# fdb/frequensea

Hardware: AMD Instinct MI355X
Metric: fft_frames_per_sec_n8192 (higher is better)
Workload: dtype f32

## Files before the change

### frequensea_amd/csrc/fsea_fft_core.h

```cpp
#pragma once

#include <hip/hip_runtime.h>
#include <stddef.h>
#include <stdint.h>

#include <fsea_pk_asm.h>
#include "fsea_opt.h"
#ifdef FSEA_TUNE
#include <fsea_pk_asm_tune.h>
#endif

namespace fsea {

constexpr int ilog2c(int n) {
    int l = 0;
    while ((1 << l) < n) ++l;
    return l;
}

constexpr int bitrev_c(int i, int bits) {
    int r = 0;
    for (int b = 0; b < bits; ++b) {
        if (i & (1 << b)) r |= 1 << (bits - 1 - b);
    }
// ... 187 lines not shown
#endif

template <int N_, int T_, int FPW_, int WPE_, int NP_, int R0_, int R1_, int R2_ = 1, int R3_ = 1,
          bool TWL_ = true, bool TWR_ = true, int ABL_ = 0, int OPT_ = FSEA_DEFAULT_OPT>
struct FftCfg {
    static constexpr int OPT = OPT_;
    static constexpr int ABL = ABL_;
    static constexpr int N = N_, T = T_, FPW = FPW_, NP = NP_;
    static constexpr int WPE = WPE_;
    static constexpr int P = N_ / T_;
    static constexpr int WG = T_ * FPW_;
    static constexpr bool TWL = TWL_, TWR = TWR_;
    static constexpr int R(int i) { return i == 0 ? R0_ : i == 1 ? R1_ : i == 2 ? R2_ : R3_; }
    static constexpr int C(int i) { return P / R(i); }
    static constexpr int Ns(int i) { return i == 0 ? 1 : Ns(i - 1) * R(i - 1); }
    static constexpr int tw_len(int i) { return i == 0 ? 0 : (R(i) - 1) * Ns(i); }
    static constexpr int pad(int idx) { return lds_pad<N_ / T_>(idx); }
    static constexpr int LDS_FRAME = N_ + 2 * T_;
    static constexpr int lds_tw_off(int i) {
        return i <= 1 ? FPW_ * LDS_FRAME : lds_tw_off(i - 1) + tw_len(i - 1);
    }
    static constexpr int TAB_MID = lds_tw_off(NP_ - 1) - FPW_ * LDS_FRAME;
    static constexpr int TAB_HI = N_ >= 64 ? N_ / 64 : 1, TAB_LO = 64;
    static constexpr int TAB_SMALL = TAB_MID + (TWR_ ? TAB_HI + TAB_LO : 0);
    static constexpr int LDS_HI = FPW_ * LDS_FRAME + TAB_MID;
    static constexpr int LDS_LO = LDS_HI + TAB_HI;
    static constexpr int LDS_TOTAL = FPW_ * LDS_FRAME + ((TWL_ || TWR_) ? TAB_SMALL : 0);
    static constexpr int LDS_ALLOC = LDS_TOTAL + 2;
    static_assert(R0_ * R1_ * R2_ * R3_ == N_, "radices must multiply to N");
    static_assert(N_ % T_ == 0, "T must divide N");
    static_assert(NP_ >= 2 && NP_ <= 4, "2..4 passes");
};

struct FftArgs {
    const void *in;
    void *out;
    size_t n_frames;
    size_t hop;
    uint32_t xormask;
    int mode;
    unsigned *ctr;
    unsigned long long *trace;
    const cf *tw[4];
    const cf *tw_small;
    const cf *tw_def;
    double rot_delta, rot_phase0;
    cf rot_row[32];
    uint32_t tile_rows = 0, pitch_row = 0, pitch_tile = 0;
    size_t out_span = 0;
    uint32_t dynamic_units = 1;
    uint32_t run_len = 0;
    const float *win = nullptr;
    const cf *win_dc = nullptr;
    uint32_t win_offset = 0;
};

template <int C>
__device__ __forceinline__ void ld_c(const cf *p, cf *dst) {
    if constexpr (C == 1) {
        dst[0] = *p;
    } else {
#pragma unroll
        for (int c = 0; c < C; c += 2) {
            const cf2 q = *reinterpret_cast<const cf2 *>(p + c);
            dst[c] = cf{q[0], q[1]};
            dst[c + 1] = cf{q[2], q[3]};
        }
    }
}

template <int C>
__device__ __forceinline__ void st_c(cf *p, const cf *src) {
    if constexpr (C == 1) {
        *p = src[0];
    } else {
#pragma unroll
        for (int c = 0; c < C; c += 2) {
            *reinterpret_cast<cf2 *>(p + c) = cf2{src[c][0], src[c][1], src[c + 1][0], src[c + 1][1]};
        }
    }
}

typedef __amdgpu_buffer_rsrc_t rsrc_t;

__device__ __forceinline__ rsrc_t buffer_window(const void *base, size_t off, size_t total) {
    const size_t rem = total > off ? total - off : 0;
    char *p = const_cast<char *>(static_cast<const char *>(base)) + (rem ? off : 0);
    return __builtin_amdgcn_make_buffer_rsrc(p, 0, rem > 0xffffffffull ? 0xffffffffu : (uint32_t)rem, 0x00020000);
// ... 517 lines not shown
            const auto q = __builtin_amdgcn_raw_buffer_load_b128(rs, voff, (uint32_t)(16 * T * i), 0);
            wv[2 * i] = cf{u2f(q[0]), u2f(q[1])};
            wv[2 * i + 1] = cf{u2f(q[2]), u2f(q[3])};
        }
    }
    static constexpr bool BALANCE = WIN == 0 && !LATE_LOAD && !ROT && IN == IN_U8 &&
                                    (((MODE_T == MODE_DB5_U8_DCFIX || MODE_T == MODE_DB10_U8) && (Cfg::OPT & opt::BALANCE_PX) != 0) ||
                                     (MODE_T == MODE_MAG && (Cfg::OPT & opt::BALANCE_MAG) != 0));
    static constexpr int BALANCE_STORES = 32;
    static __device__ __forceinline__ void balance_vmcnt() {
        if constexpr (BALANCE) {
            const rsrc_t nowhere = buffer_window(nullptr, 0, 0);
#pragma unroll
            for (int i = 0; i < BALANCE_STORES; ++i) {
                __builtin_amdgcn_raw_buffer_store_b32(0u, nowhere, (uint32_t)(64 * i), 0u, 0);
            }
        }
    }
    template <bool OFFSET>
    static __device__ __forceinline__ void convert_windowed(const Raw *raw, uint32_t xormask, int t, cf *v) {
#pragma unroll
        for (int r = 0; r < R0; ++r) convert_row<IN, C0, false, OFFSET>(raw[r], OFFSET ? xormask ^ 0x80808080u : xormask, C0 * t, v + r * C0);
    }
    template <int C = 0>
    static __device__ __forceinline__ void pass0_windowed(cf *v, const cf *wv) {
        if constexpr (C < C0) {
            dft_regs_win<R0, C0, C>(v + C, wv);
            pass0_windowed<C + 1>(v, wv);
        }
    }

#ifdef FSEA_TUNE
#include "fsea_fft_tune_members.h"
    static __device__ __forceinline__ void run(const FftArgs &a, cf *lds_all) {
        if constexpr (W64) run_w64(a, lds_all);
        else if constexpr (V2) run_v2(a, lds_all);
        else run_v1(a, lds_all);
    }
#else
    static __device__ __forceinline__ void run(const FftArgs &a, cf *lds_all) { run_v1(a, lds_all); }
#endif

    static __device__ __forceinline__ void run_v1(const FftArgs &a, cf *lds_all) {
        const int tid = threadIdx.x;
        const int slot = (FPW == 1) ? 0 : tid / T;
        const int t = (FPW == 1) ? tid : tid % T;
        cf *lds = lds_all + slot * Cfg::LDS_FRAME;
        unsigned *tk = reinterpret_cast<unsigned *>(lds_all + Cfg::LDS_TOTAL);

        const unsigned b = blockIdx.x;
        const bool issuer = (tid == 0);
        const size_t n_units = RUNS ? (a.n_frames + a.run_len - 1) / a.run_len : (a.n_frames + FPW - 1) / FPW;
        Pools pools;
        pools.n_units = (unsigned)n_units;
        pools.grid = gridDim.x;
        unsigned cur = b % POOLS;

        if ((FSEA_TRACE != 0) && a.trace != nullptr && tid == 0) {
            const unsigned hw_id = read_hw_id(), xcc_id = read_xcc_id();
            a.trace[32 * b + 0] = wall_clock64();
            a.trace[32 * b + 2] = __builtin_readcyclecounter();
            a.trace[32 * b + 4] = hw_id;
            a.trace[32 * b + 5] = xcc_id;
        }

        const int mode = (MODE_T >= 0) ? MODE_T : a.mode;
        const uint32_t xormask = (MODE_T >= 0) ? 0u : a.xormask;
        const uint32_t esz = elem_bytes(mode);
        const size_t total_in = (size_t)IN_BPS * ((a.n_frames - 1) * a.hop + (size_t)N);
        const bool tiled = a.tile_rows != 0;
        const size_t total_out = (size_t)esz * (tiled ? a.out_span : a.n_frames * (size_t)N);
        const uint32_t in_voff = (uint32_t)IN_BPS * ((uint32_t)slot * (uint32_t)a.hop + (uint32_t)(C0 * t));
        const int tl = pass_lane<LAST>(t);
        const uint32_t out_elem = (uint32_t)slot * (tiled ? a.pitch_row : (uint32_t)N) + (uint32_t)(CL * tl);
        auto row_elem = [&](size_t f) -> size_t {
            if (!tiled) return f * (size_t)N;
            const uint32_t k = (uint32_t)f / a.tile_rows, y = (uint32_t)f - k * a.tile_rows;
            return (size_t)y * a.pitch_row + (size_t)k * a.pitch_tile;
        };

        size_t u = b;
#if FSEA_STATIC_CONTIG
        [[maybe_unused]] const size_t contig_per = (n_units + gridDim.x - 1) / gridDim.x;
        [[maybe_unused]] size_t contig_end = n_units;
        if constexpr (!RUNS) {
            u = (size_t)b * contig_per;
            contig_end = u + contig_per < n_units ? u + contig_per : n_units;
            if (u >= n_units) u = n_units;
        }
#endif
        unsigned tick_next = 0;
        const bool dyn = !RUNS && DYNAMIC && a.dynamic_units != 0;
        [[maybe_unused]] size_t fcur = RUNS ? (size_t)b * a.run_len : 0;
        [[maybe_unused]] unsigned jpos = 0;
        if (dyn) {
            u = (size_t)pools.start(cur) + b / POOLS;
            if (u >= pools.start(cur + 1)) u = n_units;
        }
        constexpr int TAB_COPY = (Cfg::TWL || Cfg::TWR) ? Cfg::TAB_SMALL : 0;
        constexpr int TAB_REGS = (TAB_COPY + Cfg::WG - 1) / Cfg::WG;
        cf tabv[TAB_REGS > 0 ? TAB_REGS : 1];
#pragma unroll
        for (int i = 0; i < TAB_REGS; ++i) {
            const int e = tid + i * Cfg::WG;
            tabv[i] = a.tw_small[e < TAB_COPY ? e : TAB_COPY - 1];
        }
        constexpr int R1 = Cfg::R(1), C1 = Cfg::C(1), Ns1 = Cfg::Ns(1);
        cf tw1[DEFER ? C1 * (R1 / 2) : 1];
        if constexpr (DEFER) {
            const int t1 = pass_lane<1>(t);
#pragma unroll
            for (int c = 0; c < C1; ++c) ld_c<R1 / 2>(a.tw_def + ((C1 * t1 + c) % Ns1) * (R1 / 2), tw1 + c * (R1 / 2));
        }
        [[maybe_unused]] const rsrc_t win_rs = buffer_window(WIN ? a.win : nullptr, 0, WIN ? (size_t)N * 4u : 0);
        cf wv[WPAIRS];
        cf dcv[(WIN_DC && !DC_IN_REGS) ? DC_REGS : 1];
        cf dcr[DC_IN_REGS ? 2 * CL : 1];
        if constexpr (DC_IN_REGS) {
#pragma unroll
            for (int c = 0; c < CL; ++c) {
                dcr[c] = a.win_dc[CL * tl + c];
                dcr[CL + c] = a.win_dc[NsL + CL * tl + c];
            }
        }
        if constexpr (WIN != 0) load_window(win_rs, t, wv);
        if constexpr (WIN_DC && !DC_IN_REGS) {
#pragma unroll
            for (int i = 0; i < DC_REGS; ++i) {
                const int e = tid + i * Cfg::WG;
                dcv[i] = a.win_dc[e < 2 * NsL ? e : 2 * NsL - 1];
            }
        }
        if (dyn) {
            if (issuer) tick_next = atomicAdd(a.ctr + 32 * cur, 1u);
        }
        Raw raw[R0];
        load_raw(buffer_window(a.in, (size_t)IN_BPS * (RUNS ? fcur : u * FPW) * a.hop, u < n_units ? total_in : 0), in_voff, raw);
        balance_vmcnt();

        if constexpr (TAB_COPY > 0) {
#pragma unroll
            for (int i = 0; i < TAB_REGS; ++i) {
                const int e = tid + i * Cfg::WG;
                lds_all[FPW * Cfg::LDS_FRAME + (e < TAB_COPY ? e : TAB_COPY - 1)] = tabv[i];
            }
            if constexpr (WIN_DC && !DC_IN_REGS) {
#pragma unroll
                for (int i = 0; i < DC_REGS; ++i) {
                    const int e = tid + i * Cfg::WG;
                    lds_all[DC_OFF + (e < 2 * NsL ? e : 2 * NsL - 1)] = dcv[i];
                }
            }
            if ((FSEA_TRACE != 0) && a.trace != nullptr && tid == 0) a.trace[32 * b + 28] = wall_clock64();
            __syncthreads();
            if ((FSEA_TRACE != 0) && a.trace != nullptr && tid == 0) a.trace[32 * b + 29] = wall_clock64();
        }
        cf twl[Cfg::TWR ? (RL - 1) * CL : 1];
        if constexpr (Cfg::TWR) {
            const cf *hi = lds_all + Cfg::LDS_HI, *lo = lds_all + Cfg::LDS_LO;
            auto root = [&](unsigned m) -> cf { return pk_cmul(hi[m >> 6], lo[m & 63u]); };
            constexpr int RB = RL >= 16 ? 8 : (RL >= 4 ? 2 : RL);
            constexpr int RA = RL / RB;
#pragma unroll
            for (int c = 0; c < CL; ++c) {
                const unsigned k = (unsigned)(CL * tl + c);
                cf wb[RB], wa[RA];
#pragma unroll
                for (int bb = 1; bb < RB; ++bb) wb[bb] = root((unsigned)bb * k);
#pragma unroll
                for (int aa = 1; aa < RA; ++aa) wa[aa] = root((unsigned)(RB * aa) * k);
#pragma unroll
// ... 62 lines not shown
                    convert_row<IN, C0, false>(raw[r], a.xormask, C0 * t, v + r * C0);
                    const cf wr = a.rot_row[r];
#pragma unroll
                    for (int c = 0; c < C0; ++c) {
                        v[r * C0 + c] = pk_cmul(v[r * C0 + c] + cf{128.0f, 128.0f}, pk_cmul_uniform(fr[c], wr));
                        if constexpr (WIN != 0) {
                            if (a.win_offset != 0) v[r * C0 + c] += cf{128.0f, 128.0f};
                        }
                    }
                }
            } else if constexpr (WIN != 0 && IN == IN_F32) {
#pragma unroll
                for (int r = 0; r < R0; ++r) convert_row<IN, C0, false>(raw[r], 0u, C0 * t, v + r * C0);
            } else if constexpr (WIN != 0) {
                if (a.win_offset != 0) convert_windowed<true>(raw, xormask, t, v);
                else convert_windowed<false>(raw, xormask, t, v);
            } else {
#pragma unroll
                for (int r = 0; r < R0; ++r) convert_row<IN, C0>(raw[r], xormask, C0 * t, v + r * C0);
            }
            if ((FSEA_TRACE != 0) && a.trace != nullptr && tid == 0 && iter == 0) {
                asm volatile("" ::"v"(v[0]));
                a.trace[32 * b + 30] = wall_clock64();
            }
            if constexpr (WIN != 0) {
                pass0_windowed(v, wv);
            } else {
#pragma unroll
                for (int c = 0; c < C0; ++c) dft_regs<R0, C0, (Cfg::ABL & abl::NO_FLOPS) != 0>(v + c);
            }
            lds_write<0>(lds, v, t);
            frame_sync();
            if ((FSEA_TRACE != 0) && a.trace != nullptr && tid == 0 && iter == 0) a.trace[32 * b + 7] = wall_clock64();
            size_t un = u + gridDim.x;
#if FSEA_STATIC_CONTIG
            if constexpr (!RUNS) un = u + 1 < contig_end ? u + 1 : n_units;
#endif
            [[maybe_unused]] size_t fnext = 0;
            [[maybe_unused]] bool same_run = false;
            if constexpr (RUNS) {
                same_run = (jpos + 1 < a.run_len) && (fcur + 1 < a.n_frames);
                un = same_run ? u : u + gridDim.x;
                fnext = same_run ? fcur + 1 : un * (size_t)a.run_len;
            }
            if (dyn) {
                if constexpr (Cfg::ABL & abl::NO_LDS) __syncthreads();
                const unsigned nu = __builtin_amdgcn_readfirstlane(tk[par]);
                par ^= 1u;
                un = (nu == NO_UNIT) ? n_units : (size_t)nu;
            }
            if constexpr (RUNS) {
                const rsrc_t rs = buffer_window(a.in, (size_t)IN_BPS * fnext * a.hop, un < n_units ? total_in : 0);
                if (same_run) {
#pragma unroll
                    for (int r = 0; r < R0 / 2; ++r) raw[r] = raw[r + R0 / 2];
                    load_raw_rows<R0 / 2, R0>(rs, in_voff, raw);
                } else {
                    load_raw(rs, in_voff, raw);
                }
            } else if constexpr ((Cfg::ABL & abl::NO_LOADS) == 0 && !LATE_LOAD) {
                load_raw(buffer_window(a.in, (size_t)IN_BPS * (un * FPW) * a.hop, un < n_units ? total_in : 0), in_voff, raw);
            }
            middle_pass<1>(lds, lds_all, v, a, t, tw1);

            lds_read<LAST>(lds, v, tl);
            after_reads();
            frame_sync();
            if constexpr (Cfg::TWR && TW_FUSE) {
#pragma unroll
                for (int c = 0; c < CL; ++c) dft_regs_tw<RL, CL, CL>(v + c, twl + c, PRESCALED ? SC : 1.0f);
            } else if constexpr (Cfg::TWR) {
                if constexpr (PRESCALED) {
#pragma unroll
                    for (int c = 0; c < CL; ++c) v[c] = v[c] * cf{SC, SC};
                }
// ... 25 lines not shown
                for (int c = 0; c < CL; c += CB) {
                    cf dc_lo[CB], dc_hi[CB];
                    ld_c<CB>(lds_all + DC_OFF + CL * tl + c, dc_lo);
                    ld_c<CB>(lds_all + DC_OFF + NsL + CL * tl + c, dc_hi);
#pragma unroll
                    for (int j = 0; j < CB; ++j) {
                        v[(RL / 2 - 1) * CL + c + j] += dc_lo[j];
                        v[(RL / 2) * CL + c + j] += dc_hi[j];
                    }
                }
            }
            if constexpr (WIN != 0) {
                if constexpr (WIN == 1) {
                    load_window(win_rs, t, wv);
                    __builtin_amdgcn_sched_barrier(0);
                }
            }
            epilogue(mode, buffer_window(a.out, (size_t)esz * row_elem(RUNS ? fcur : u * FPW), total_out), out_elem, v, tl);
            if constexpr (LATE_LOAD) {
                load_raw(buffer_window(a.in, (size_t)IN_BPS * (un * FPW) * a.hop, un < n_units ? total_in : 0), in_voff, raw);
            }
            u = un;
            if constexpr (RUNS) {
                fcur = fnext;
                jpos = same_run ? jpos + 1 : 0;
            }
            if ((FSEA_TRACE != 0) && a.trace != nullptr && tid == 0 && iter < 24) a.trace[32 * b + 8 + iter] = wall_clock64();
            ++iter;
        }

        if (dyn && issuer) {
            __builtin_amdgcn_s_waitcnt(0);
            const unsigned finished = atomicAdd(a.ctr + 32 * POOLS, 1u);
            if (finished == gridDim.x - 1) {
#pragma unroll
                for (unsigned q = 0; q <= POOLS; ++q) a.ctr[32 * q] = 0;
            }
        }
        if ((FSEA_TRACE != 0) && a.trace != nullptr && tid == 0) {
            a.trace[32 * b + 1] = wall_clock64();
            a.trace[32 * b + 3] = __builtin_readcyclecounter();
        }
    }
};

}
```

### frequensea_amd/csrc/fsea_fft_tune_members.h

```cpp
    static __device__ __forceinline__ void run_w64(const FftArgs &a, cf *lds) {
        static_assert(!W64 || (N == 4096 && T == 64 && FPW == 1 && NP == 2 && R0 == 64 && RL == 64), "W64 is the 64 x 64 layout");
        static_assert(!W64 || (IN == IN_U8 && !ROT), "W64 serves the u8 kernels");
        static_assert(!W64 || (!Cfg::TWL && !Cfg::TWR), "W64 keeps its (deferred) twiddles in registers: no table block in LDS");
        constexpr int ROW = 66;
        const int L = threadIdx.x;
        const unsigned b = blockIdx.x;
        const size_t n_units = a.n_frames;
        const int mode = (MODE_T >= 0) ? MODE_T : a.mode;
        const uint32_t xormask = (MODE_T >= 0) ? 0u : a.xormask;
        const uint32_t esz = elem_bytes(mode);
        const size_t total_in = (size_t)IN_BPS * ((a.n_frames - 1) * a.hop + (size_t)N);
        const bool tiled = a.tile_rows != 0;
        const size_t total_out = (size_t)esz * (tiled ? a.out_span : a.n_frames * (size_t)N);
        auto row_elem = [&](size_t f) -> size_t {
            if (!tiled) return f * (size_t)N;
            const uint32_t k = (uint32_t)f / a.tile_rows, y = (uint32_t)f - k * a.tile_rows;
            return (size_t)y * a.pitch_row + (size_t)k * a.pitch_tile;
        };
        const int t5 = L & 31, odd = L & 1, hi = L >> 5;
        const int pi = (t5 & 16) + ((t5 & 15) >> 1) + 8 * odd;
        const int n2 = 2 * pi + (hi ^ odd);
        const uint32_t in_voff = 4u * (uint32_t)(pi + 32 * hi);
        const uint32_t sel_a = odd ? 0x07060302u : 0x05040100u;
        const uint32_t sel_b = odd ? 0x05040100u : 0x07060302u;
        cf twd[RL / 2];
        ld_c<RL / 2>(a.tw_def + (size_t)L * (RL / 2), twd);

        auto load_frame = [&](size_t u, uint32_t *raw) {
            const rsrc_t rs = buffer_window(a.in, (size_t)IN_BPS * u * a.hop, u < n_units ? total_in : 0);
#pragma unroll
            for (int j = 0; j < 32; ++j) raw[j] = __builtin_amdgcn_raw_buffer_load_b32(rs, in_voff, (uint32_t)(256 * j), LD_AUX);
        };
        size_t u = b;
        uint32_t raw[32];
        load_frame(u, raw);
        unsigned grid_v = gridDim.x;
#if defined(__AMDGCN__)
        asm volatile("" : "+v"(grid_v));
#endif
        cf *const wr = lds + n2;
        const cf *const rd = lds + ROW * L;

        while (u < n_units) {
            cf v[64];
#pragma unroll
            for (int j = 0; j < 16; ++j) {
                uint32_t wa = byte_perm(raw[j + 16], raw[j], sel_a);
                uint32_t wb = byte_perm(raw[j + 16], raw[j], sel_b);
                lane_swap32(wa, wb);
                wa ^= xormask;
                wb ^= xormask;
                v[2 * j] = cf{s8f(wa, 0), s8f(wa, 1)};
                v[2 * j + 32] = cf{s8f(wa, 2), s8f(wa, 3)};
                v[2 * j + 1] = cf{s8f(wb, 0), s8f(wb, 1)};
                v[2 * j + 33] = cf{s8f(wb, 2), s8f(wb, 3)};
            }
            dft_regs<64, 1, (Cfg::ABL & abl::NO_FLOPS) != 0>(v);
            frame_sync();
            if constexpr ((Cfg::ABL & abl::NO_LDS) == 0) {
#pragma unroll
                for (int k1 = 0; k1 < 64; ++k1) wr[ROW * k1] = v[k1];
            }
            frame_sync();
            const size_t un = u + __builtin_amdgcn_readfirstlane(grid_v);
            if constexpr ((Cfg::ABL & abl::NO_LOADS) == 0) load_frame(un, raw);
            if constexpr ((Cfg::ABL & abl::NO_LDS) == 0) {
#pragma unroll
                for (int q = 0; q < 16; ++q) {
                    ld_c<2>(rd + 2 * q, v + 2 * q);
// ... 20 lines not shown
        const uint32_t sel1 = (L & 1) ? 0x03070105u : 0x06020400u;
        const uint32_t sel2 = (L & 2) ? 0x03020706u : 0x05040100u;
        const uint32_t voff = (uint32_t)((L & 3) * 64 + (L & ~3));
        uint32_t left = 0;
#pragma unroll
        for (int q = 0; q < 16; ++q) {
            uint32_t px = 0;
#pragma unroll
            for (int i = 0; i < 4; ++i) {
                const cf z = w[4 * q + i];
                const float p = __builtin_fmaf(z[0], z[0], z[1] * z[1]);
                float d = __builtin_fmaf(kdb, __builtin_amdgcn_logf(p), PX_BIAS ? koff - 0.49999997f : koff);
                if constexpr (Cfg::ABL & abl::NO_EPILOGUE_MATH) d = kdb * p;
                px = cvt_pk_u8(PX_BIAS ? d : trunc_f32(d), (uint32_t)i, px);
            }
            const uint32_t u1 = byte_perm(quad_xor1(px), px, sel1);
            uint32_t rows = byte_perm(quad_xor2(u1), u1, sel2);
            if (q == 7) left = read_lane(rows, 63) >> 24;
            if (q == 8 && patched && L == 0) rows = (rows & 0xffffff00u) | left;
            if constexpr (Cfg::ABL & abl::NO_STORES) {
                if (rows == 0x01020304u && w[0][0] == -1.0f) __builtin_amdgcn_raw_buffer_store_b32(rows, out, voff, (uint32_t)(256 * q), ST_AUX);
            } else {
                __builtin_amdgcn_raw_buffer_store_b32(rows, out, voff, (uint32_t)(256 * q), ST_AUX);
            }
        }
    }

    static __device__ __forceinline__ void wave_order() {
        __builtin_amdgcn_fence(__ATOMIC_RELEASE, "wavefront");
        __builtin_amdgcn_wave_barrier();
        __builtin_amdgcn_fence(__ATOMIC_ACQUIRE, "wavefront");
    }

    static __device__ __forceinline__ void run_v2(const FftArgs &a, cf *lds_all) {
        constexpr int RA = Cfg::R(0), RB = Cfg::R(1), RC = Cfg::R(2);
        static_assert(NP == 3 && FPW == 1 && (T % 64) == 0 && !ONE_WAVE, "V2 is for multi-wave frames in three passes");
        static_assert(RA == 16 && RB == 16 && RC == 32 && P == 32, "V2 layout constants are written for 16 x 16 x 32");
        static_assert(Cfg::TWR, "V2 keeps the last pass's twiddles in registers");
        constexpr int G = 64 / RB;
        constexpr int ROW_B = RC / 2 + 1;
        constexpr int SW = 64 * ROW_B;
        constexpr int ROW_A = 4 * RB + 1;
        static_assert((RA - 1) * ROW_A + 16 * (G - 1) + RB <= SW, "the A layout must fit the wave's partition");
        static_assert(2 * SW * (T / 64) <= Cfg::LDS_FRAME, "LDS frame too small for the B layout");

        const int tid = threadIdx.x;
        const int w = tid >> 6, l = tid & 63;
        unsigned *tk = reinterpret_cast<unsigned *>(lds_all + Cfg::LDS_TOTAL);
        cf *lds = lds_all;

        const unsigned bidx = blockIdx.x;
        const bool issuer = (tid == 0);
        const size_t n_units = a.n_frames;
        Pools pools;
        pools.n_units = (unsigned)n_units;
        pools.grid = gridDim.x;
        unsigned cur = bidx % POOLS;

        if ((FSEA_TRACE != 0) && a.trace != nullptr && tid == 0) {
            const unsigned hw_id = read_hw_id(), xcc_id = read_xcc_id();
            a.trace[32 * bidx + 0] = wall_clock64();
            a.trace[32 * bidx + 2] = __builtin_readcyclecounter();
            a.trace[32 * bidx + 4] = hw_id;
            a.trace[32 * bidx + 5] = xcc_id;
        }

        const int mode = (MODE_T >= 0) ? MODE_T : a.mode;
        const uint32_t xormask = (MODE_T >= 0) ? 0u : a.xormask;
        const uint32_t esz = elem_bytes(mode);
        const size_t total_in = (size_t)IN_BPS * ((a.n_frames - 1) * a.hop + (size_t)N);
        const bool tiled = a.tile_rows != 0;
        const size_t total_out = (size_t)esz * (tiled ? a.out_span : a.n_frames * (size_t)N);
        auto row_elem = [&](size_t f) -> size_t {
            if (!tiled) return f * (size_t)N;
            const uint32_t k = (uint32_t)f / a.tile_rows, y = (uint32_t)f - k * a.tile_rows;
            return (size_t)y * a.pitch_row + (size_t)k * a.pitch_tile;
        };
        const int b0 = l % RB, g = l / RB;
        const int n_base = b0 * RC + (w * G + g) * C0;
        const uint32_t in_voff = (uint32_t)IN_BPS * (uint32_t)((Cfg::ABL & abl::V2_V1_LOADS) ? C0 * tid : n_base);
        constexpr bool STATIC = (Cfg::ABL & abl::V2_STATIC) != 0;
        const int ka = l % RA;
        const int m = tid;
        const uint32_t out_elem = (uint32_t)m;

        size_t u = (size_t)pools.start(cur) + bidx / POOLS;
        if (u >= pools.start(cur + 1)) u = n_units;
        if constexpr (STATIC) u = bidx;
        unsigned tick_next = 0;
// ... 69 lines not shown
        if ((FSEA_TRACE != 0) && a.trace != nullptr && tid == 0) a.trace[32 * bidx + 6] = wall_clock64();
        while (u < n_units) {
            if (!STATIC && issuer) {
                unsigned nu = pools.unit(cur, tick_next);
                for (unsigned k = 1; nu == NO_UNIT && k < POOLS; ++k) {
                    const unsigned q = (cur + k) % POOLS;
                    nu = pools.unit(q, atomicAdd(a.ctr + 32 * q, 1u));
                    if (nu != NO_UNIT) cur = q;
                }
                tk[par] = nu;
                tick_next = atomicAdd(a.ctr + 32 * cur, 1u);
            }

            cf v[P];
            if constexpr (ROT) {
                const size_t first = u * a.hop;
                const cf ef = turn_phasor_f32(a.rot_phase0 + a.rot_delta * (double)first);
                cf fr[C0];
#pragma unroll
                for (int c = 0; c < C0; ++c) fr[c] = pk_cmul(ebase[c], ef);
#pragma unroll
                for (int r = 0; r < R0; ++r) {
                    convert_row<IN, C0, false>(raw[r], a.xormask, n_base, v + r * C0);
                    const cf wr = a.rot_row[r];
#pragma unroll
                    for (int c = 0; c < C0; ++c) {
                        v[r * C0 + c] = pk_cmul(v[r * C0 + c] + cf{128.0f, 128.0f}, pk_cmul_uniform(fr[c], wr));
                    }
                }
            } else {
#pragma unroll
                for (int r = 0; r < R0; ++r) convert_row<IN, C0>(raw[r], xormask, n_base, v + r * C0);
            }
            size_t un = u + gridDim.x;
            if constexpr (STATIC) {
                load_raw(buffer_window(a.in, (size_t)IN_BPS * un * a.hop, un < n_units ? total_in : 0), in_voff, raw);
            }
#pragma unroll
            for (int c = 0; c < C0; ++c) dft_regs<R0, C0>(v + c);

            if constexpr ((Cfg::ABL & abl::V2_NO_EXCHANGE_A) == 0) {
                wave_order();
#pragma unroll
                for (int r = 0; r < RA; ++r) st_c<2>(a_wr + 2 * ROW_A * r, v + 2 * r);
                wave_order();
#pragma unroll
                for (int r = 0; r < RB; ++r) ld_c<2>(a_rd + 2 * r, v + 2 * r);
                after_reads();
            }
#pragma unroll
            for (int c = 0; c < 2; ++c) dft_regs_def<RB, 2, 1>(v + c, tw1);

            __syncthreads();
            if ((FSEA_TRACE != 0) && a.trace != nullptr && tid == 0 && iter == 0) a.trace[32 * bidx + 7] = wall_clock64();
#pragma unroll
            for (int r = 0; r < RB; ++r) st_c<2>(b_wr + 2 * ROW_B * RA * r, v + 2 * r);
            __syncthreads();
            const unsigned tkv = STATIC ? 0u : tk[par];
#pragma unroll
            for (int j = 0; j < RC / 2; ++j) ld_c<2>(b_rd + 2 * j, v + 2 * j);
            if constexpr (!STATIC) {
                __builtin_amdgcn_sched_barrier(0);
                const unsigned nu = __builtin_amdgcn_readfirstlane(tkv);
                par ^= 1u;
                un = (nu == NO_UNIT) ? n_units : (size_t)nu;
                load_raw(buffer_window(a.in, (size_t)IN_BPS * un * a.hop, un < n_units ? total_in : 0), in_voff, raw);
            }
            after_reads();

            if constexpr (TW_FUSE) {
                dft_regs_tw<RL, 1, 1>(v, twl, PRESCALED ? SC : 1.0f);
            } else {
                if constexpr (PRESCALED) v[0] = v[0] * cf{SC, SC};
#pragma unroll
                for (int r = 1; r < RL; ++r) v[r] = pk_cmul(v[r], twl[r - 1]);
                dft_regs<RL, 1>(v);
            }
            epilogue(mode, buffer_window(a.out, (size_t)esz * row_elem(u), total_out), out_elem, v, m);
            u = un;
            if ((FSEA_TRACE != 0) && a.trace != nullptr && tid == 0 && iter < 24) a.trace[32 * bidx + 8 + iter] = wall_clock64();
            ++iter;
        }

        if (!STATIC && issuer) {
            __builtin_amdgcn_s_waitcnt(0);
            const unsigned finished = atomicAdd(a.ctr + 32 * POOLS, 1u);
            if (finished == gridDim.x - 1) {
#pragma unroll
                for (unsigned q = 0; q <= POOLS; ++q) a.ctr[32 * q] = 0;
            }
        }
        if ((FSEA_TRACE != 0) && a.trace != nullptr && tid == 0) {
            a.trace[32 * bidx + 1] = wall_clock64();
            a.trace[32 * bidx + 3] = __builtin_readcyclecounter();
        }
    }
```

### frequensea_amd/csrc/fsea_plan.hip

```cpp
#include "../../include/fsea.h"

#include <hip/hip_runtime.h>

#include <cmath>
#include <cstdlib>
#include <cstring>
#include <mutex>
#include <string>
#include <vector>

#include "fsea_registry.h"
#include "fsea_tables.h"
#include "fsea_internal.h"

using namespace fsea_detail;

extern "C" int fsea_kernels_small(fsea::KernelEntry *out, int cap);
extern "C" int fsea_kernels_alt(fsea::KernelEntry *out, int cap);
extern "C" int fsea_kernels_1024(fsea::KernelEntry *out, int cap);
extern "C" int fsea_kernels_2048(fsea::KernelEntry *out, int cap);
extern "C" int fsea_kernels_4096(fsea::KernelEntry *out, int cap);
extern "C" int fsea_kernels_8192(fsea::KernelEntry *out, int cap);
extern "C" int fsea_kernels_16384(fsea::KernelEntry *out, int cap);
#ifdef FSEA_TUNE
// ... 79 lines not shown
    return nullptr;
}

int select_kind(const fsea_plan *p, int in_kind, int mode, int flip) {
    const fsea::KernelEntry *e = p->entry;
    int kind = fsea::K_U8;
    if (in_kind == fsea::IN_F32) kind = fsea::K_F32;
    else if (in_kind == fsea::IN_U8_ROT) kind = fsea::K_U8_ROT;
    else if (flip && mode == FSEA_MODE_MAG_F32) kind = fsea::K_U8_MAG;
    else if (flip && mode == FSEA_MODE_DB5_U8_DCFIX) kind = fsea::K_U8_DB5;
    else if (flip && mode == FSEA_MODE_DB10_U8) kind = fsea::K_U8_DB10;
    if (p->window.form != 0) {
        static const int twin[] = {fsea::K_U8_MAG_WIN, fsea::K_U8_DB5_WIN, fsea::K_U8_DB10_WIN,
                                   fsea::K_U8_WIN,     fsea::K_U8_ROT_WIN, fsea::K_F32_WIN};
        kind = twin[kind];
    }
    if (!e->fn[kind] && in_kind == fsea::IN_U8) kind = p->window.form != 0 ? fsea::K_U8_WIN : fsea::K_U8;
    if (!e->fn[kind]) {
        fail(FSEA_EINVAL, "kernel variant '%s' has no entry point for this input kind", e->variant);
        return -1;
    }
    return kind;
}

int half_overlap_kind(const fsea_plan *p, int kind, size_t n_frames, bool tiled) {
    const int half = kind == fsea::K_U8_MAG ? fsea::K_U8_MAG_HALF : kind == fsea::K_U8_MAG_WIN ? fsea::K_U8_MAG_HALF_WIN : -1;
    if (half < 0 || !p->entry->fn[half] || tiled || n_frames < 2 || 2 * (size_t)p->hop != (size_t)p->n || p->no_half_overlap) {
        return -1;
    }
    return half;
}

void launch_kind(const fsea::KernelEntry *e, int kind, fsea::FftArgs &a, unsigned grid, hipStream_t s) {
    void *args[] = {&a};
    (void)hipLaunchKernel(e->fn[kind], dim3(grid), dim3(e->wg), args, 0, s);
}

__global__ void fsea_sum_f32_kernel(const float *x, size_t n, double *acc) {
    double s = 0.0;
    for (size_t i = (size_t)blockIdx.x * blockDim.x + threadIdx.x; i < n; i += (size_t)gridDim.x * blockDim.x) {
        s += (double)x[i];
    }
    for (int off = 32; off > 0; off >>= 1) s += __shfl_down(s, off, 64);
    __shared__ double part[16];
    const int lane = threadIdx.x & 63, w = threadIdx.x >> 6;
    if (lane == 0) part[w] = s;
    __syncthreads();
    if (threadIdx.x == 0) {
        double tot = 0.0;
        for (int i = 0; i < (int)(blockDim.x >> 6); ++i) tot += part[i];
        atomicAdd(acc, tot);
    }
}

std::string pow2_kernel_name(const fsea_plan *p) {
    const int k = select_kind(p, fsea::IN_U8, p->mode, 1);
    if (k < 0) return "";
    const int half = half_overlap_kind(p, k, 2, false);
    return p->entry->name[half >= 0 ? half : k];
}

unsigned grid_for(const fsea_plan *p, const fsea::KernelEntry *e, int occ, size_t n_frames) {
    const size_t units = (n_frames + e->fpw - 1) / e->fpw;
    size_t g = (size_t)p->num_cu * (size_t)(occ > 0 ? occ : 1);
    if (units < g) g = units;
    if (g >= 8) g &= ~(size_t)7;
    if (g == 0) g = 1;
// ... 31 lines not shown
            } else {
                (void)hipGetLastError();
                if (oldest < 0 || c.seq < p->ctr.slots[oldest].seq) oldest = (int)i;
            }
        }
        if (pick < 0 && oldest >= 0) {
            if (hipEventSynchronize(p->ctr.slots[oldest].ev) != hipSuccess) return nullptr;
            pick = oldest;
        }
        if (pick < 0) return nullptr;
        p->ctr.slots[pick].used = true;
        p->ctr.slots[pick].pending = false;
        p->ctr.slots[pick].anonymous = anonymous;
        p->ctr.slots[pick].stream = s;
    }
    fsea_plan::Counters::Slot &c = p->ctr.slots[pick];
    if (capturing) c.captured = true;
    if (!capturing && !c.ev) {
        if (c.ev.create() != hipSuccess) return nullptr;
    }
    c.seq = ++p->ctr.slot_seq;
    c.launching = true;
    *index = pick;
    *record = !capturing;
    return p->ctr.d_ctr.ptr + (size_t)FSEA_CTR_WORDS * (size_t)pick;
}

int launch_pow2(fsea_plan *p, int in_kind, const void *d_in, size_t n_frames, int flip, int mode, void *d_out,
                hipStream_t s, double rot_delta, double rot_phase0, const TileLayout *tiles) {
    if (n_frames == 0) return FSEA_OK;
    const int kind = select_kind(p, in_kind, mode, flip);
    if (kind < 0) return FSEA_EINVAL;
    const fsea::KernelEntry *e = p->entry;
    fsea::FftArgs a;
    a.win = p->window.d_win.ptr;
    a.win_dc = p->window.d_win_dc.ptr;
    a.win_offset = p->window.form == 2 ? 1u : 0u;
    a.rot_delta = rot_delta;
    a.rot_phase0 = rot_phase0;
    if (in_kind == fsea::IN_U8_ROT) {
        fsea::TwPair rows[32];
        fsea::build_rotation_rows(p->n, e->radix[0], rot_delta, rows);
        for (int r = 0; r < 32; ++r) a.rot_row[r] = fsea::cf{rows[r].re, rows[r].im};
    }
    a.in = d_in;
    a.out = d_out;
    a.n_frames = n_frames;
    a.hop = (size_t)p->hop;
    a.xormask = flip ? 0u : 0x80808080u;
    a.mode = mode;
    a.trace = p->d_trace.ptr;
    for (int i = 0; i < 4; ++i) a.tw[i] = p->d_tw.ptr + p->tw_off[i];
    a.tw_small = p->d_tw.ptr;
    a.tw_def = p->d_tw.ptr + p->tw_def_off;
    {
        const unsigned grid = grid_for(p, e, p->occ[kind], n_frames);
        const size_t n_units = (n_frames + (size_t)e->fpw - 1) / (size_t)e->fpw;
        a.dynamic_units = p->units_policy == FSEA_UNITS_TICKETS  ? 1u
                          : p->units_policy == FSEA_UNITS_STATIC ? 0u
                                                                 : (n_units > (size_t)FSEA_STATIC_UNITS_PER_WG * grid ? 1u : 0u);
    }
    if (tiles) {
        a.tile_rows = tiles->rows;
        a.pitch_row = tiles->pitch_row;
        a.pitch_tile = tiles->pitch_tile;
        a.out_span = tiles->span;
// ... 495 lines not shown
```

### frequensea_amd/csrc/fsea_registry.h

```cpp
#pragma once

#include <hip/hip_runtime.h>
#include <stddef.h>

#include "fsea_fft_core.h"

namespace fsea {

enum : int { K_U8_MAG = 0, K_U8_DB5 = 1, K_U8_DB10 = 2, K_U8 = 3, K_U8_ROT = 4, K_F32 = 5, K_U8_MAG_HALF = 6,
             K_U8_MAG_WIN = 7, K_U8_WIN = 8, K_U8_MAG_HALF_WIN = 9, K_U8_DB5_WIN = 10, K_U8_DB10_WIN = 11,
             K_U8_ROT_WIN = 12, K_F32_WIN = 13, K_COUNT = 14 };

struct KernelEntry {
    int n;
    const char *variant;
    int t, fpw, wg, np;
    int radix[4];
    int c0;
    int counters;
    const void *fn[K_COUNT];
    const char *name[K_COUNT];
    size_t lds_bytes[K_COUNT];
};

inline bool add_kind(KernelEntry &e, int kind, const void *fn, const char *name, size_t lds_bytes) {
    e.fn[kind] = fn;
    e.name[kind] = name;
    e.lds_bytes[kind] = lds_bytes;
    return true;
}


}

#define FSEA_KERNEL_FN_(NAME, SUFFIX, ...)                                                            \
    extern "C" __global__ __launch_bounds__(NAME##_cfg::WG, NAME##_cfg::WPE) void NAME##SUFFIX(       \
        fsea::FftArgs a) {                                                                            \
        __shared__ __attribute__((aligned(16))) fsea::cf lds[fsea::FftKernel<NAME##_cfg, __VA_ARGS__>::LDS_CF]; \
        fsea::FftKernel<NAME##_cfg, __VA_ARGS__>::run(a, lds);                                        \
    }

#define FSEA_KIND_(NAME, KIND, SUFFIX, ...)                                                           \
    FSEA_KERNEL_FN_(NAME, SUFFIX, __VA_ARGS__)                                                        \
    [[maybe_unused]] static const bool NAME##SUFFIX##_added = fsea::add_kind(                         \
        NAME##_entry, fsea::KIND, reinterpret_cast<const void *>(&NAME##SUFFIX), #NAME #SUFFIX,       \
        sizeof(fsea::cf) * fsea::FftKernel<NAME##_cfg, __VA_ARGS__>::LDS_CF);

#define FSEA_K_U8_MAG_(N)             FSEA_KIND_(N, K_U8_MAG,          _u8_mag,          fsea::IN_U8,  fsea::MODE_MAG,          false, false, 0)
#define FSEA_K_U8_DB5_(N)             FSEA_KIND_(N, K_U8_DB5,          _u8_db5,          fsea::IN_U8,  fsea::MODE_DB5_U8_DCFIX, false, false, 0)
#define FSEA_K_U8_DB10_(N)            FSEA_KIND_(N, K_U8_DB10,         _u8_db10,         fsea::IN_U8,  fsea::MODE_DB10_U8,      false, false, 0)
#define FSEA_K_U8_(N)                 FSEA_KIND_(N, K_U8,              _u8,              fsea::IN_U8,  -1,                      false, false, 0)
#define FSEA_K_U8_ROT_(N)             FSEA_KIND_(N, K_U8_ROT,          _u8_rot,          fsea::IN_U8,  -1,                      true,  false, 0)
#define FSEA_K_F32_(N)                FSEA_KIND_(N, K_F32,             _f32,             fsea::IN_F32, -1,                      false, false, 0)
#define FSEA_K_U8_MAG_HALF_(N)        FSEA_KIND_(N, K_U8_MAG_HALF,     _u8_mag_half,     fsea::IN_U8,  fsea::MODE_MAG,          false, true,  0)
#define FSEA_K_U8_MAG_WIN_(N, W)      FSEA_KIND_(N, K_U8_MAG_WIN,      _u8_mag_win,      fsea::IN_U8,  fsea::MODE_MAG,          false, false, W)
#define FSEA_K_U8_DB5_WIN_(N, W)      FSEA_KIND_(N, K_U8_DB5_WIN,      _u8_db5_win,      fsea::IN_U8,  fsea::MODE_DB5_U8_DCFIX, false, false, W)
#define FSEA_K_U8_DB10_WIN_(N, W)     FSEA_KIND_(N, K_U8_DB10_WIN,     _u8_db10_win,     fsea::IN_U8,  fsea::MODE_DB10_U8,      false, false, W)
#define FSEA_K_U8_WIN_(N, W)          FSEA_KIND_(N, K_U8_WIN,          _u8_win,          fsea::IN_U8,  -1,                      false, false, W)
#define FSEA_K_U8_ROT_WIN_(N, W)      FSEA_KIND_(N, K_U8_ROT_WIN,      _u8_rot_win,      fsea::IN_U8,  -1,                      true,  false, W)
#define FSEA_K_F32_WIN_(N, W)         FSEA_KIND_(N, K_F32_WIN,         _f32_win,         fsea::IN_F32, -1,                      false, false, W)
#define FSEA_K_U8_MAG_HALF_WIN_(N, W) FSEA_KIND_(N, K_U8_MAG_HALF_WIN, _u8_mag_half_win, fsea::IN_U8,  fsea::MODE_MAG,          false, true,  W)

#define FSEA_CONFIG_(NAME, VARIANT, ...)                                                              \
    using NAME##_cfg = fsea::FftCfg<__VA_ARGS__>;                                                     \
    static fsea::KernelEntry NAME##_entry = {                                                         \
        NAME##_cfg::N, VARIANT, NAME##_cfg::T, NAME##_cfg::FPW, NAME##_cfg::WG, NAME##_cfg::NP,       \
        {NAME##_cfg::R(0), NAME##_cfg::R(1), NAME##_cfg::R(2), NAME##_cfg::R(3)}, NAME##_cfg::C(0),   \
        fsea::FftKernel<NAME##_cfg, fsea::IN_U8>::counters_used()};

#define FSEA_DEFINE_KERNEL(NAME, VARIANT, ...)                                                        \
    FSEA_CONFIG_(NAME, VARIANT, __VA_ARGS__)                                                          \
    FSEA_K_U8_MAG_(NAME) FSEA_K_U8_DB5_(NAME) FSEA_K_U8_DB10_(NAME) FSEA_K_U8_(NAME) FSEA_K_U8_ROT_(NAME) FSEA_K_F32_(NAME)

#define FSEA_DEFINE_KERNEL_LITE(NAME, VARIANT, ...)                                                   \
    FSEA_CONFIG_(NAME, VARIANT, __VA_ARGS__)                                                          \
    FSEA_K_U8_MAG_(NAME) FSEA_K_U8_(NAME)

#define FSEA_DEFINE_KERNEL_U8(NAME, VARIANT, ...)                                                     \
    FSEA_CONFIG_(NAME, VARIANT, __VA_ARGS__)                                                          \
    FSEA_K_U8_MAG_(NAME) FSEA_K_U8_DB5_(NAME) FSEA_K_U8_DB10_(NAME) FSEA_K_U8_(NAME)

#define FSEA_DEFINE_HALF_OVERLAP(NAME) FSEA_K_U8_MAG_HALF_(NAME)

#define FSEA_DEFINE_WINDOWED(NAME, WMODE)                                                             \
    FSEA_K_U8_MAG_WIN_(NAME, WMODE) FSEA_K_U8_DB5_WIN_(NAME, WMODE) FSEA_K_U8_DB10_WIN_(NAME, WMODE)  \
    FSEA_K_U8_WIN_(NAME, WMODE) FSEA_K_U8_ROT_WIN_(NAME, WMODE) FSEA_K_F32_WIN_(NAME, WMODE)
#define FSEA_DEFINE_HALF_OVERLAP_WIN(NAME, WMODE) FSEA_K_U8_MAG_HALF_WIN_(NAME, WMODE)

#define FSEA_REGISTER_BEGIN(TAG)                                                                      \
    extern "C" int fsea_kernels_##TAG(fsea::KernelEntry *out, int cap) {                              \
        int n = 0;
#define FSEA_REGISTER(NAME) if (n < cap) out[n++] = NAME##_entry;
#define FSEA_REGISTER_END                                                                             \
        return n;                                                                                     \
// ... 2 lines not shown
```

Measured before the change: 83.93 million.

## Split kernel arguments into hot scalars and cold struct, pass grid explicitly

Replaces the single large FftArgs kernel argument with nine hot scalar parameters, a 128-byte cold struct, and a rotation-row block passed only to the rotation kernels. This shrinks the kernarg segment and puts the most-used fields first so they load early. The grid size now comes in as an argument instead of gridDim.x, and the twiddle register loads are hoisted ahead of the unit scheduling. Trace stores move after the first input load. It also narrows n_frames and hop to 32 bits and adds a host check that rejects more than 2^32-1 frames.

After: 83.81 million (median of 2 runs). About the same (-0.2%).

```diff
diff --git a/frequensea_amd/csrc/fsea_fft_core.h b/frequensea_amd/csrc/fsea_fft_core.h
--- a/frequensea_amd/csrc/fsea_fft_core.h
+++ b/frequensea_amd/csrc/fsea_fft_core.h
@@ -243,28 +243,63 @@
     static_assert(NP_ >= 2 && NP_ <= 4, "2..4 passes");
 };
 
-struct FftArgs {
-    const void *in;
-    void *out;
-    size_t n_frames;
-    size_t hop;
+struct alignas(64) FftCold {
+    size_t out_span = 0;
+    uint32_t tile_rows = 0, pitch_row = 0;
     uint32_t xormask;
     int mode;
-    unsigned *ctr;
-    unsigned long long *trace;
-    const cf *tw[4];
-    const cf *tw_small;
-    const cf *tw_def;
-    double rot_delta, rot_phase0;
-    cf rot_row[32];
-    uint32_t tile_rows = 0, pitch_row = 0, pitch_tile = 0;
-    size_t out_span = 0;
-    uint32_t dynamic_units = 1;
-    uint32_t run_len = 0;
+    uint32_t pad0_ = 0;
+    uint32_t pitch_tile = 0;
     const float *win = nullptr;
     const cf *win_dc = nullptr;
     uint32_t win_offset = 0;
+    uint32_t pad1_ = 0;
+    unsigned long long *trace;
+    const cf *tw[4];
+    double rot_delta, rot_phase0;
 };
+static_assert(sizeof(FftCold) == 128 && offsetof(FftCold, tw) == 64, "the cold arguments are two cache lines");
+
+struct FftRot {
+    cf rot_row[32];
+};
+
+struct FftArgs : FftCold {
+    const void *in;
+    const cf *tw_small;
+    unsigned *ctr;
+    size_t n_frames;
+    size_t hop;
+    uint32_t dynamic_units = 1;
+    uint32_t run_len = 0;
+    const cf *tw_def;
+    void *out;
+    cf rot_row[32];
+};
+
+#define FSEA_HOT_PARAMS_                                                                                      \
+    const void *in, const fsea::cf *tw_small, unsigned *ctr, uint32_t n_frames, uint32_t hop, uint32_t grid,  \
+        uint32_t units, const fsea::cf *tw_def, void *out
+#define FSEA_HOT_COUNT_ 9
+__device__ __forceinline__ FftArgs make_args(FSEA_HOT_PARAMS_, const FftCold &cold, const FftRot *rot) {
+    (void)grid;
+    FftArgs a;
+    static_cast<FftCold &>(a) = cold;
+    a.in = in;
+    a.tw_small = tw_small;
+    a.ctr = ctr;
+    a.n_frames = n_frames;
+    a.hop = hop;
+    a.dynamic_units = units;
+    a.run_len = units;
+    a.tw_def = tw_def;
+    a.out = out;
+    if (rot != nullptr) {
+#pragma unroll
+        for (int r = 0; r < 32; ++r) a.rot_row[r] = rot->rot_row[r];
+    }
+    return a;
+}
 
 template <int C>
 __device__ __forceinline__ void ld_c(const cf *p, cf *dst) {
@@ -848,16 +883,17 @@
 
 #ifdef FSEA_TUNE
 #include "fsea_fft_tune_members.h"
-    static __device__ __forceinline__ void run(const FftArgs &a, cf *lds_all) {
-        if constexpr (W64) run_w64(a, lds_all);
-        else if constexpr (V2) run_v2(a, lds_all);
-        else run_v1(a, lds_all);
+    static __device__ __forceinline__ void run(const FftArgs &a, cf *lds_all, unsigned grid) {
+        if constexpr (W64) run_w64(a, lds_all, grid);
+        else if constexpr (V2) run_v2(a, lds_all, grid);
+        else run_v1(a, lds_all, grid);
     }
 #else
-    static __device__ __forceinline__ void run(const FftArgs &a, cf *lds_all) { run_v1(a, lds_all); }
+    static __device__ __forceinline__ void run(const FftArgs &a, cf *lds_all, unsigned grid) { run_v1(a, lds_all, grid); }
 #endif
-
-    static __device__ __forceinline__ void run_v1(const FftArgs &a, cf *lds_all) {
+    static __device__ __forceinline__ void run(const FftArgs &a, cf *lds_all) { run(a, lds_all, gridDim.x); }
+
+    static __device__ __forceinline__ void run_v1(const FftArgs &a, cf *lds_all, const unsigned grid) {
         const int tid = threadIdx.x;
         const int slot = (FPW == 1) ? 0 : tid / T;
         const int t = (FPW == 1) ? tid : tid % T;
@@ -869,16 +905,28 @@
         const size_t n_units = RUNS ? (a.n_frames + a.run_len - 1) / a.run_len : (a.n_frames + FPW - 1) / FPW;
         Pools pools;
         pools.n_units = (unsigned)n_units;
-        pools.grid = gridDim.x;
+        pools.grid = grid;
         unsigned cur = b % POOLS;
 
-        if ((FSEA_TRACE != 0) && a.trace != nullptr && tid == 0) {
-            const unsigned hw_id = read_hw_id(), xcc_id = read_xcc_id();
-            a.trace[32 * b + 0] = wall_clock64();
-            a.trace[32 * b + 2] = __builtin_readcyclecounter();
-            a.trace[32 * b + 4] = hw_id;
-            a.trace[32 * b + 5] = xcc_id;
-        }
+        [[maybe_unused]] const unsigned long long t_wall0 = (FSEA_TRACE != 0) ? wall_clock64() : 0ull;
+        [[maybe_unused]] const unsigned long long t_clk0 = (FSEA_TRACE != 0) ? __builtin_readcyclecounter() : 0ull;
+
+        constexpr int TAB_COPY = (Cfg::TWL || Cfg::TWR) ? Cfg::TAB_SMALL : 0;
+        constexpr int TAB_REGS = (TAB_COPY + Cfg::WG - 1) / Cfg::WG;
+        cf tabv[TAB_REGS > 0 ? TAB_REGS : 1];
+#pragma unroll
+        for (int i = 0; i < TAB_REGS; ++i) {
+            const int e = tid + i * Cfg::WG;
+            tabv[i] = a.tw_small[e < TAB_COPY ? e : TAB_COPY - 1];
+        }
+        constexpr int R1 = Cfg::R(1), C1 = Cfg::C(1), Ns1 = Cfg::Ns(1);
+        cf tw1[DEFER ? C1 * (R1 / 2) : 1];
+        if constexpr (DEFER) {
+            const int t1 = pass_lane<1>(t);
+#pragma unroll
+            for (int c = 0; c < C1; ++c) ld_c<R1 / 2>(a.tw_def + ((C1 * t1 + c) % Ns1) * (R1 / 2), tw1 + c * (R1 / 2));
+        }
+        if constexpr (WIN != 0) __builtin_amdgcn_sched_barrier(0);
 
         const int mode = (MODE_T >= 0) ? MODE_T : a.mode;
         const uint32_t xormask = (MODE_T >= 0) ? 0u : a.xormask;
@@ -897,7 +945,7 @@
 
         size_t u = b;
 #if FSEA_STATIC_CONTIG
-        [[maybe_unused]] const size_t contig_per = (n_units + gridDim.x - 1) / gridDim.x;
+        [[maybe_unused]] const size_t contig_per = (n_units + grid - 1) / grid;
         [[maybe_unused]] size_t contig_end = n_units;
         if constexpr (!RUNS) {
             u = (size_t)b * contig_per;
@@ -913,21 +961,6 @@
             u = (size_t)pools.start(cur) + b / POOLS;
             if (u >= pools.start(cur + 1)) u = n_units;
         }
-        constexpr int TAB_COPY = (Cfg::TWL || Cfg::TWR) ? Cfg::TAB_SMALL : 0;
-        constexpr int TAB_REGS = (TAB_COPY + Cfg::WG - 1) / Cfg::WG;
-        cf tabv[TAB_REGS > 0 ? TAB_REGS : 1];
-#pragma unroll
-        for (int i = 0; i < TAB_REGS; ++i) {
-            const int e = tid + i * Cfg::WG;
-            tabv[i] = a.tw_small[e < TAB_COPY ? e : TAB_COPY - 1];
-        }
-        constexpr int R1 = Cfg::R(1), C1 = Cfg::C(1), Ns1 = Cfg::Ns(1);
-        cf tw1[DEFER ? C1 * (R1 / 2) : 1];
-        if constexpr (DEFER) {
-            const int t1 = pass_lane<1>(t);
-#pragma unroll
-            for (int c = 0; c < C1; ++c) ld_c<R1 / 2>(a.tw_def + ((C1 * t1 + c) % Ns1) * (R1 / 2), tw1 + c * (R1 / 2));
-        }
         [[maybe_unused]] const rsrc_t win_rs = buffer_window(WIN ? a.win : nullptr, 0, WIN ? (size_t)N * 4u : 0);
         cf wv[WPAIRS];
         cf dcv[(WIN_DC && !DC_IN_REGS) ? DC_REGS : 1];
@@ -953,6 +986,13 @@
         Raw raw[R0];
         load_raw(buffer_window(a.in, (size_t)IN_BPS * (RUNS ? fcur : u * FPW) * a.hop, u < n_units ? total_in : 0), in_voff, raw);
         balance_vmcnt();
+        if ((FSEA_TRACE != 0) && a.trace != nullptr && tid == 0) {
+            const unsigned hw_id = read_hw_id(), xcc_id = read_xcc_id();
+            a.trace[32 * b + 0] = t_wall0;
+            a.trace[32 * b + 2] = t_clk0;
+            a.trace[32 * b + 4] = hw_id;
+            a.trace[32 * b + 5] = xcc_id;
+        }
 
         if constexpr (TAB_COPY > 0) {
 #pragma unroll
@@ -1081,7 +1121,7 @@
             lds_write<0>(lds, v, t);
             frame_sync();
             if ((FSEA_TRACE != 0) && a.trace != nullptr && tid == 0 && iter == 0) a.trace[32 * b + 7] = wall_clock64();
-            size_t un = u + gridDim.x;
+            size_t un = u + grid;
 #if FSEA_STATIC_CONTIG
             if constexpr (!RUNS) un = u + 1 < contig_end ? u + 1 : n_units;
 #endif
@@ -1089,7 +1129,7 @@
             [[maybe_unused]] bool same_run = false;
             if constexpr (RUNS) {
                 same_run = (jpos + 1 < a.run_len) && (fcur + 1 < a.n_frames);
-                un = same_run ? u : u + gridDim.x;
+                un = same_run ? u : u + grid;
                 fnext = same_run ? fcur + 1 : un * (size_t)a.run_len;
             }
             if (dyn) {
@@ -1181,7 +1221,7 @@
         if (dyn && issuer) {
             __builtin_amdgcn_s_waitcnt(0);
             const unsigned finished = atomicAdd(a.ctr + 32 * POOLS, 1u);
-            if (finished == gridDim.x - 1) {
+            if (finished == grid - 1) {
 #pragma unroll
                 for (unsigned q = 0; q <= POOLS; ++q) a.ctr[32 * q] = 0;
             }
diff --git a/frequensea_amd/csrc/fsea_fft_tune_members.h b/frequensea_amd/csrc/fsea_fft_tune_members.h
--- a/frequensea_amd/csrc/fsea_fft_tune_members.h
+++ b/frequensea_amd/csrc/fsea_fft_tune_members.h
@@ -1,4 +1,4 @@
-    static __device__ __forceinline__ void run_w64(const FftArgs &a, cf *lds) {
+    static __device__ __forceinline__ void run_w64(const FftArgs &a, cf *lds, const unsigned grid) {
         static_assert(!W64 || (N == 4096 && T == 64 && FPW == 1 && NP == 2 && R0 == 64 && RL == 64), "W64 is the 64 x 64 layout");
         static_assert(!W64 || (IN == IN_U8 && !ROT), "W64 serves the u8 kernels");
         static_assert(!W64 || (!Cfg::TWL && !Cfg::TWR), "W64 keeps its (deferred) twiddles in registers: no table block in LDS");
@@ -34,7 +34,7 @@
         size_t u = b;
         uint32_t raw[32];
         load_frame(u, raw);
-        unsigned grid_v = gridDim.x;
+        unsigned grid_v = grid;
 #if defined(__AMDGCN__)
         asm volatile("" : "+v"(grid_v));
 #endif
@@ -121,7 +121,7 @@
         __builtin_amdgcn_fence(__ATOMIC_ACQUIRE, "wavefront");
     }
 
-    static __device__ __forceinline__ void run_v2(const FftArgs &a, cf *lds_all) {
+    static __device__ __forceinline__ void run_v2(const FftArgs &a, cf *lds_all, const unsigned grid) {
         constexpr int RA = Cfg::R(0), RB = Cfg::R(1), RC = Cfg::R(2);
         static_assert(NP == 3 && FPW == 1 && (T % 64) == 0 && !ONE_WAVE, "V2 is for multi-wave frames in three passes");
         static_assert(RA == 16 && RB == 16 && RC == 32 && P == 32, "V2 layout constants are written for 16 x 16 x 32");
@@ -143,7 +143,7 @@
         const size_t n_units = a.n_frames;
         Pools pools;
         pools.n_units = (unsigned)n_units;
-        pools.grid = gridDim.x;
+        pools.grid = grid;
         unsigned cur = bidx % POOLS;
 
         if ((FSEA_TRACE != 0) && a.trace != nullptr && tid == 0) {
@@ -279,7 +279,7 @@
 #pragma unroll
                 for (int r = 0; r < R0; ++r) convert_row<IN, C0>(raw[r], xormask, n_base, v + r * C0);
             }
-            size_t un = u + gridDim.x;
+            size_t un = u + grid;
             if constexpr (STATIC) {
                 load_raw(buffer_window(a.in, (size_t)IN_BPS * un * a.hop, un < n_units ? total_in : 0), in_voff, raw);
             }
@@ -332,7 +332,7 @@
         if (!STATIC && issuer) {
             __builtin_amdgcn_s_waitcnt(0);
             const unsigned finished = atomicAdd(a.ctr + 32 * POOLS, 1u);
-            if (finished == gridDim.x - 1) {
+            if (finished == grid - 1) {
 #pragma unroll
                 for (unsigned q = 0; q <= POOLS; ++q) a.ctr[32 * q] = 0;
             }
diff --git a/frequensea_amd/csrc/fsea_plan.hip b/frequensea_amd/csrc/fsea_plan.hip
--- a/frequensea_amd/csrc/fsea_plan.hip
+++ b/frequensea_amd/csrc/fsea_plan.hip
@@ -135,7 +135,12 @@
 }
 
 void launch_kind(const fsea::KernelEntry *e, int kind, fsea::FftArgs &a, unsigned grid, hipStream_t s) {
-    void *args[] = {&a};
+    uint32_t n_frames = (uint32_t)a.n_frames, hop = (uint32_t)a.hop;
+    uint32_t units = (kind == fsea::K_U8_MAG_HALF || kind == fsea::K_U8_MAG_HALF_WIN) ? a.run_len : a.dynamic_units;
+    fsea::FftCold *cold = &a;
+    void *args[FSEA_HOT_COUNT_ + 2] = {&a.in,   &a.tw_small, &a.ctr,    &n_frames, &hop,
+                                       &grid,   &units,      &a.tw_def, &a.out,    cold,
+                                       a.rot_row};
     (void)hipLaunchKernel(e->fn[kind], dim3(grid), dim3(e->wg), args, 0, s);
 }
 
@@ -233,6 +238,7 @@
     const int kind = select_kind(p, in_kind, mode, flip);
     if (kind < 0) return FSEA_EINVAL;
     const fsea::KernelEntry *e = p->entry;
+    if (n_frames > 0xffffffffull) return fail(FSEA_EINVAL, "n_frames %zu: a launch takes at most 2^32 - 1 frames", n_frames);
     fsea::FftArgs a;
     a.win = p->window.d_win.ptr;
     a.win_dc = p->window.d_win_dc.ptr;
diff --git a/frequensea_amd/csrc/fsea_registry.h b/frequensea_amd/csrc/fsea_registry.h
--- a/frequensea_amd/csrc/fsea_registry.h
+++ b/frequensea_amd/csrc/fsea_registry.h
@@ -33,33 +33,39 @@
 
 }
 
-#define FSEA_KERNEL_FN_(NAME, SUFFIX, ...)                                                            \
+#define FSEA_ROT_PARAM_0
+#define FSEA_ROT_PARAM_1 , fsea::FftRot rot
+#define FSEA_ROT_ROWS_0 nullptr
+#define FSEA_ROT_ROWS_1 &rot
+#define FSEA_KERNEL_FN_(NAME, SUFFIX, ISROT, ...)                                                     \
     extern "C" __global__ __launch_bounds__(NAME##_cfg::WG, NAME##_cfg::WPE) void NAME##SUFFIX(       \
-        fsea::FftArgs a) {                                                                            \
+        FSEA_HOT_PARAMS_, fsea::FftCold cold FSEA_ROT_PARAM_##ISROT) {                                \
         __shared__ __attribute__((aligned(16))) fsea::cf lds[fsea::FftKernel<NAME##_cfg, __VA_ARGS__>::LDS_CF]; \
-        fsea::FftKernel<NAME##_cfg, __VA_ARGS__>::run(a, lds);                                        \
+        fsea::FftKernel<NAME##_cfg, __VA_ARGS__>::run(                                                \
+            fsea::make_args(in, tw_small, ctr, n_frames, hop, grid, units, tw_def, out, cold,         \
+                            FSEA_ROT_ROWS_##ISROT), lds, grid);                                       \
     }
 
-#define FSEA_KIND_(NAME, KIND, SUFFIX, ...)                                                           \
-    FSEA_KERNEL_FN_(NAME, SUFFIX, __VA_ARGS__)                                                        \
+#define FSEA_KIND_(NAME, KIND, SUFFIX, ISROT, ...)                                                    \
+    FSEA_KERNEL_FN_(NAME, SUFFIX, ISROT, __VA_ARGS__)                                                 \
     [[maybe_unused]] static const bool NAME##SUFFIX##_added = fsea::add_kind(                         \
         NAME##_entry, fsea::KIND, reinterpret_cast<const void *>(&NAME##SUFFIX), #NAME #SUFFIX,       \
         sizeof(fsea::cf) * fsea::FftKernel<NAME##_cfg, __VA_ARGS__>::LDS_CF);
 
-#define FSEA_K_U8_MAG_(N)             FSEA_KIND_(N, K_U8_MAG,          _u8_mag,          fsea::IN_U8,  fsea::MODE_MAG,          false, false, 0)
-#define FSEA_K_U8_DB5_(N)             FSEA_KIND_(N, K_U8_DB5,          _u8_db5,          fsea::IN_U8,  fsea::MODE_DB5_U8_DCFIX, false, false, 0)
-#define FSEA_K_U8_DB10_(N)            FSEA_KIND_(N, K_U8_DB10,         _u8_db10,         fsea::IN_U8,  fsea::MODE_DB10_U8,      false, false, 0)
-#define FSEA_K_U8_(N)                 FSEA_KIND_(N, K_U8,              _u8,              fsea::IN_U8,  -1,                      false, false, 0)
-#define FSEA_K_U8_ROT_(N)             FSEA_KIND_(N, K_U8_ROT,          _u8_rot,          fsea::IN_U8,  -1,                      true,  false, 0)
-#define FSEA_K_F32_(N)                FSEA_KIND_(N, K_F32,             _f32,             fsea::IN_F32, -1,                      false, false, 0)
-#define FSEA_K_U8_MAG_HALF_(N)        FSEA_KIND_(N, K_U8_MAG_HALF,     _u8_mag_half,     fsea::IN_U8,  fsea::MODE_MAG,          false, true,  0)
-#define FSEA_K_U8_MAG_WIN_(N, W)      FSEA_KIND_(N, K_U8_MAG_WIN,      _u8_mag_win,      fsea::IN_U8,  fsea::MODE_MAG,          false, false, W)
-#define FSEA_K_U8_DB5_WIN_(N, W)      FSEA_KIND_(N, K_U8_DB5_WIN,      _u8_db5_win,      fsea::IN_U8,  fsea::MODE_DB5_U8_DCFIX, false, false, W)
-#define FSEA_K_U8_DB10_WIN_(N, W)     FSEA_KIND_(N, K_U8_DB10_WIN,     _u8_db10_win,     fsea::IN_U8,  fsea::MODE_DB10_U8,      false, false, W)
-#define FSEA_K_U8_WIN_(N, W)          FSEA_KIND_(N, K_U8_WIN,          _u8_win,          fsea::IN_U8,  -1,                      false, false, W)
-#define FSEA_K_U8_ROT_WIN_(N, W)      FSEA_KIND_(N, K_U8_ROT_WIN,      _u8_rot_win,      fsea::IN_U8,  -1,                      true,  false, W)
-#define FSEA_K_F32_WIN_(N, W)         FSEA_KIND_(N, K_F32_WIN,         _f32_win,         fsea::IN_F32, -1,                      false, false, W)
-#define FSEA_K_U8_MAG_HALF_WIN_(N, W) FSEA_KIND_(N, K_U8_MAG_HALF_WIN, _u8_mag_half_win, fsea::IN_U8,  fsea::MODE_MAG,          false, true,  W)
+#define FSEA_K_U8_MAG_(N)             FSEA_KIND_(N, K_U8_MAG,          _u8_mag,          0,   fsea::IN_U8,  fsea::MODE_MAG,          false, false, 0)
+#define FSEA_K_U8_DB5_(N)             FSEA_KIND_(N, K_U8_DB5,          _u8_db5,          0,   fsea::IN_U8,  fsea::MODE_DB5_U8_DCFIX, false, false, 0)
+#define FSEA_K_U8_DB10_(N)            FSEA_KIND_(N, K_U8_DB10,         _u8_db10,         0,   fsea::IN_U8,  fsea::MODE_DB10_U8,      false, false, 0)
+#define FSEA_K_U8_(N)                 FSEA_KIND_(N, K_U8,              _u8,              0,   fsea::IN_U8,  -1,                      false, false, 0)
+#define FSEA_K_U8_ROT_(N)             FSEA_KIND_(N, K_U8_ROT,          _u8_rot,          1,   fsea::IN_U8,  -1,                      true,  false, 0)
+#define FSEA_K_F32_(N)                FSEA_KIND_(N, K_F32,             _f32,             0,   fsea::IN_F32, -1,                      false, false, 0)
+#define FSEA_K_U8_MAG_HALF_(N)        FSEA_KIND_(N, K_U8_MAG_HALF,     _u8_mag_half,     0,   fsea::IN_U8,  fsea::MODE_MAG,          false, true,  0)
+#define FSEA_K_U8_MAG_WIN_(N, W)      FSEA_KIND_(N, K_U8_MAG_WIN,      _u8_mag_win,      0,   fsea::IN_U8,  fsea::MODE_MAG,          false, false, W)
+#define FSEA_K_U8_DB5_WIN_(N, W)      FSEA_KIND_(N, K_U8_DB5_WIN,      _u8_db5_win,      0,   fsea::IN_U8,  fsea::MODE_DB5_U8_DCFIX, false, false, W)
+#define FSEA_K_U8_DB10_WIN_(N, W)     FSEA_KIND_(N, K_U8_DB10_WIN,     _u8_db10_win,     0,   fsea::IN_U8,  fsea::MODE_DB10_U8,      false, false, W)
+#define FSEA_K_U8_WIN_(N, W)          FSEA_KIND_(N, K_U8_WIN,          _u8_win,          0,   fsea::IN_U8,  -1,                      false, false, W)
+#define FSEA_K_U8_ROT_WIN_(N, W)      FSEA_KIND_(N, K_U8_ROT_WIN,      _u8_rot_win,      1,   fsea::IN_U8,  -1,                      true,  false, W)
+#define FSEA_K_F32_WIN_(N, W)         FSEA_KIND_(N, K_F32_WIN,         _f32_win,         0,   fsea::IN_F32, -1,                      false, false, W)
+#define FSEA_K_U8_MAG_HALF_WIN_(N, W) FSEA_KIND_(N, K_U8_MAG_HALF_WIN, _u8_mag_half_win, 0,   fsea::IN_U8,  fsea::MODE_MAG,          false, true,  W)
 
 #define FSEA_CONFIG_(NAME, VARIANT, ...)                                                              \
     using NAME##_cfg = fsea::FftCfg<__VA_ARGS__>;                                                     \
```
